# sanderslab/magellanmapper

Hardware: AMD Instinct MI355X
Metric: Mvoxels/s, 2048x2048x1024 uint16 stack, 5-sigma LoG blob detection (higher is better)
Workload: dtype f16x2 MFMA (f32 accumulate) + 16-bit fixed-point intermediates; f64 re-score of every candidate

## Files before the change

### magellanmapper_amd/csrc/mmx_ymfma.hip

```cpp

#include <type_traits>

#include <cstdlib>

#include "mmx_device.h"

struct ym_cfg {
    float w2[MMX_MAX_RADIUS_FAST + 1];
    float w0[MMX_MAX_RADIUS_FAST + 1];
    float unscale;
    float start;
    float lo, eps;
    int radius;
    int reverse;
};

namespace {

#ifndef YM5_OCC
#define YM5_OCC 2
#endif
#ifndef YM6_WAVES
#define YM6_WAVES 4
#define YM6_JH 4
#define YM6_NF 4
#endif
template <int NB, bool MASK>
__global__ void __launch_bounds__(NB <= 4 ? 256 : YM6_WAVES * 64, NB <= 4 ? 3 : (YM6_WAVES == 4 ? YM5_OCC : 1))
ym_kernel(const mmx_block* __restrict__ blocks, int64_t slot_elems, int64_t tile_stride,
          const unsigned* __restrict__ gt, float* __restrict__ out, ym_cfg cfg,
          unsigned long long* __restrict__ mask)
{
    constexpr int RB = 8 * (NB - 2);
    constexpr int NF = NB <= 4 ? 4 : YM6_NF;
    __shared__ v4u frag[NB * NF * 64];
    constexpr int WAVES = NB <= 4 ? 4 : YM6_WAVES;
    constexpr int JH = NB <= 4 ? 4 : YM6_JH;
    __shared__ float tr[WAVES * 2 * 1024];

    const mmx_block bd = blocks[cfg.reverse ? gridDim.y - 1 - blockIdx.y : blockIdx.y];
    const int ntx = (bd.nx + 15) >> 4, ntz = (bd.nz + 15) >> 4;
    if ((int)blockIdx.x * (WAVES / 4) >= ntx * ntz) return;
    for (int e = threadIdx.x; e < NB * NF * 64; e += WAVES * 64) {
        const int ln = e & 63, f = e >> 6;
        const int piece = (f % NF) % (NF / 2), kern = (f % NF) / (NF / 2), t = f / NF;
        const int m = ln & 15, kq = ln >> 4;
        const int delta = RB - 16 * t;
        unsigned pk[4];
#pragma unroll
        for (int i = 0; i < 8; i += 2) {
            float v[2];
#pragma unroll
            for (int u = 0; u < 2; ++u) {
                int d = 8 * kq + i + u - m + delta;
                d = d < 0 ? -d : d;
                const float ws = d <= cfg.radius ? (kern ? cfg.w0[d] : cfg.w2[d]) : 0.f;
                const float h = (float)(_Float16)ws;
                v[u] = piece == 0 ? h : (piece == 1 ? (ws - h) * 256.f : h * 256.f);
            }
            pk[i >> 1] = pack_h2(v[0], v[1]);
        }
        frag[e] = (v4u){pk[0], pk[1], pk[2], pk[3]};
    }
    __syncthreads();

    const int wv = __builtin_amdgcn_readfirstlane((int)(threadIdx.x >> 6));
    const int tile = (int)blockIdx.x * (WAVES / 4) + (wv >> 2);
    if (tile >= ntx * ntz) return;
    const int c = tile / ntz, U = tile - c * ntz;
    const int zq = wv & 3;
    if (16 * U + 4 * zq >= bd.nz) return;
    const int lane = threadIdx.x & 63;
    const int n = bd.ny;
    const float nms_lo = cfg.lo, nms_eps = cfg.eps, us = cfg.unscale;
    const int kq = lane >> 4, n16 = lane & 15;
    const unsigned trow_b = (unsigned)(ntx * ntz) * 1024u;
    const rsrc_t rs = make_rsrc(gt + (int64_t)bd.slot * tile_stride + (int64_t)tile * 256);
    const unsigned voff = (unsigned)(zq * 256 + n16 * 16);
    const unsigned voff_s = voff + (unsigned)(8 * kq) * trow_b;
    const int xi = lane & 15;
    const int z = 16 * U + 4 * zq + (lane >> 4), x = 16 * c + xi;
    const bool real = z < bd.nz && x < bd.nx;
    float* w1 = out + (int64_t)bd.slot * slot_elems;
    const rsrc_t rsw = make_rsrc(w1);
    const unsigned ooff = (unsigned)((real ? z : 0) * bd.ny * bd.px + (real ? x : 0)) * 4u;
    const unsigned row_b = (unsigned)bd.px * 4u;
    const mmx_entry_geom eg = mmx_entry_geom_make(MMX_MASK_QUADS, bd.nz, bd.nx, bd.px);
    const int nent = eg.per_row;
    ulonglong2* mrow = MASK ? reinterpret_cast<ulonglong2*>(mask) + mmx_entry_base(bd.slot, slot_elems) +
                              mmx_quads_entry(eg, 4 * U + zq, 0) + c
                            : nullptr;
    unsigned long long ab_prev = 0;
    const bool has_l = xi > 0, has_r = xi < 15 && x + 1 < bd.nx;
    float prev1 = -INFINITY, prev2 = -INFINITY, nbx_prev = -INFINITY;
    int ydone = 0;
    float* trw = tr + wv * 2048;

    auto close_pending = [&]() __attribute__((always_inline)) {
        unsigned long long m = 0;
        if (ab_prev) {
            const bool cand = real & (prev1 > nms_lo) & !(fmaxf(prev2, nbx_prev) > prev1 + nms_eps);
            m = __ballot(cand);
        }
        if (lane == 0) *mrow = make_ulonglong2(m, ab_prev);
    };
    auto row = [&](float acc, int y) __attribute__((always_inline)) {
        const unsigned long long ab = MASK ? mmx_above_word(real, acc, nms_lo) : ~0ull;
#ifndef YM_NOSTORE
        if (ab && real) __builtin_amdgcn_raw_buffer_store_b32(__float_as_uint(acc * us), rsw, ooff, (unsigned)y * row_b, 0);
#endif
        if constexpr (MASK) {
            float nbx = -INFINITY;
            if (ab) {
                nbx = mmx_x_neighbours<false>(acc, has_l, has_r);
            }
            if (ydone > 0) {
                unsigned long long m = 0;
                if (ab_prev) {
                    const bool cand = real & (prev1 > nms_lo) & !(fmaxf(fmaxf(prev2, acc), nbx_prev) > prev1 + nms_eps);
                    m = __ballot(cand);
                }
                if (lane == 0) *mrow = make_ulonglong2(m, ab_prev);
                mrow += nent;
            }
            prev2 = prev1; prev1 = acc; nbx_prev = nbx;
            ab_prev = ab;
            ++ydone;
        }
    };
    auto rows_of = [&](int T, int s, bool any) __attribute__((always_inline)) {
        if (T < 0 || 16 * T >= n) return;
        const int cnt = n - 16 * T < 16 ? n - 16 * T : 16;
        if (MASK && !any) {
            if (ydone > 0) {
                close_pending();
                mrow += nent;
            }
            if (lane < cnt - 1) mrow[(int64_t)lane * nent] = make_ulonglong2(0ull, 0ull);
            mrow += (int64_t)(cnt - 1) * nent;
            prev1 = prev2 = nbx_prev = -INFINITY;
            ab_prev = 0;
            ydone += cnt;
            return;
        }
        const float* src = trw + s * 1024 + lane;
        if (!MASK || cnt < 16) {
#pragma unroll 1
            for (int r = 0; r < cnt; ++r) row(src[r * 64], 16 * T + r);
            return;
        }
        float v[16];
#pragma unroll
        for (int r = 0; r < 16; ++r) v[r] = src[r * 64];
        unsigned long long ab[16];
        unsigned long long some = 0;
#pragma unroll
        for (int r = 0; r < 16; ++r) { ab[r] = mmx_above_word(real, v[r], nms_lo); some |= ab[r]; }
        unsigned e0 = 0, e1 = 0, e2 = 0, e3 = 0;
        auto put = [&](int ln, unsigned long long m, unsigned long long a) __attribute__((always_inline)) {
            const bool me = lane == ln;
            e0 = me ? (unsigned)m : e0;
            e1 = me ? (unsigned)(m >> 32) : e1;
            e2 = me ? (unsigned)a : e2;
            e3 = me ? (unsigned)(a >> 32) : e3;
        };
        if (ab_prev) {
            const bool cand = real & (prev1 > nms_lo) & !(fmaxf(fmaxf(prev2, v[0]), nbx_prev) > prev1 + nms_eps);
            put(0, __ballot(cand), ab_prev);
        }
        float nbx15 = -INFINITY;
        if (some) {
#pragma unroll
            for (int r = 0; r < 16; ++r) {
                if (ab[r]) {
#ifndef YM_NOSTORE
                    if (real) __builtin_amdgcn_raw_buffer_store_b32(__float_as_uint(v[r] * us), rsw, ooff, (unsigned)(16 * T + r) * row_b, 0);
#endif
                    const float nbx = mmx_x_neighbours<false>(v[r], has_l, has_r);
                    if (r < 15) {
                        const float below = r > 0 ? v[r > 0 ? r - 1 : 0] : prev1;
                        const bool cand = real & (v[r] > nms_lo) & !(fmaxf(fmaxf(below, v[r < 15 ? r + 1 : 15]), nbx) > v[r] + nms_eps);
                        put(r + 1, __ballot(cand), ab[r]);
                    } else {
                        nbx15 = nbx;
                    }
                }
            }
        }
        if (lane < 16 && (lane > 0 || ydone > 0)) {
            ulonglong2* dst = mrow + (int64_t)(ydone > 0 ? lane : lane - 1) * nent;
            *dst = make_ulonglong2((unsigned long long)e0 | ((unsigned long long)e1 << 32),
                                   (unsigned long long)e2 | ((unsigned long long)e3 << 32));
        }
        mrow += (int64_t)(ydone > 0 ? 16 : 15) * nent;
        prev2 = v[14]; prev1 = v[15]; nbx_prev = nbx15;
        ab_prev = ab[15];
        ydone += 16;
    };

#ifndef YM_PFD
#define YM_PFD 1
#endif
    constexpr int PFD = YM_PFD;
    v4u rawA[8], rawB[PFD == 2 ? 8 : 1];
    auto load_block = [&](int b, v4u (&raw)[8]) __attribute__((always_inline)) {
        const int r0 = -RB + 32 * b;
        if (r0 >= 0 && r0 + 32 <= n) {
#pragma unroll
            for (int i = 0; i < 8; ++i)
                raw[i] = __builtin_bit_cast(v4u, __builtin_amdgcn_raw_buffer_load_b128(rs, voff_s, (unsigned)(r0 + i) * trow_b, 0));
        } else {
#pragma unroll
            for (int i = 0; i < 8; ++i) {
                int v = r0 + 8 * kq + i;
                v = v < 0 ? -1 - v : v;
                v = v >= n ? 2 * n - 1 - v : v;
                v = v < 0 ? 0 : (v > n - 1 ? n - 1 : v);
                raw[i] = __builtin_bit_cast(v4u, __builtin_amdgcn_raw_buffer_load_b128(rs, voff + (unsigned)v * trow_b, 0, 0));
            }
        }
    };
    const int nT = (n + 15) >> 4;
    const int nKB = (nT + NB - 3) / 2 + 1;
    const v4f start = {cfg.start, cfg.start, cfg.start, cfg.start};
    v4f acc[NB][4];
#pragma unroll
    for (int t = 0; t < NB; ++t)
#pragma unroll
        for (int j = 0; j < 4; ++j) acc[t][j] = start;
    bool any0 = false, any1 = false;

    const _Float16 k256 = (_Float16)256.f;
    auto iter = [&](int b, v4u (&raw)[8]) __attribute__((always_inline)) {
#ifndef YM_ROWS_LATE
#define YM_ROWS_LATE 1
#endif
        if (!YM_ROWS_LATE || b == nKB) {
#pragma unroll 1
            for (int h = 0; h < 2; ++h) rows_of(2 * (b - 1) - NB + 2 + h, h, h ? any1 : any0);
        }
        if (b == nKB) return false;
        if constexpr (JH < 4) { any0 = !MASK; any1 = !MASK; }
#pragma unroll
        for (int j0 = 0; j0 < 4; j0 += JH) {
            __builtin_amdgcn_sched_barrier(0);
            v4u pc[JH][4];
#pragma unroll
            for (int j = 0; j < JH; ++j)
#pragma unroll
                for (int p = 0; p < 4; ++p) {
                    const unsigned d0 = raw[2 * p][j0 + j], d1 = raw[2 * p + 1][j0 + j];
                    pc[j][0][p] = __builtin_amdgcn_perm(d1, d0, 0x0c050c01u);
                    pc[j][1][p] = __builtin_amdgcn_perm(d1, d0, 0x0c040c00u);
                    pc[j][2][p] = __builtin_amdgcn_perm(d1, d0, 0x0c070c03u) ^ 0x00800080u;
                    pc[j][3][p] = __builtin_amdgcn_perm(d1, d0, 0x0c060c02u);
                }
            __builtin_amdgcn_sched_barrier(0);
            if (j0 + JH == 4 && b + PFD < nKB) load_block(b + PFD, raw);
            __builtin_amdgcn_sched_barrier(0);
            if (YM_ROWS_LATE && JH == 4) {
#pragma unroll 1
                for (int h = 0; h < 2; ++h) rows_of(2 * (b - 1) - NB + 2 + h, h, h ? any1 : any0);
                __builtin_amdgcn_sched_barrier(0);
            }
            auto tile_mfmas = [&](int t, bool fresh) __attribute__((always_inline)) {
                v4f* a = &acc[t][j0];
                const v4u* fr = frag + (t * NF) * 64 + lane;
                const v4u ah = fr[0], al = fr[64], bh = fr[(NF / 2) * 64], bl = fr[(NF / 2 + 1) * 64];
                const v4u a256 = NF == 6 ? fr[128] : __builtin_bit_cast(v4u, __builtin_bit_cast(v8h, ah) * k256);
                const v4u b256 = NF == 6 ? fr[320] : __builtin_bit_cast(v4u, __builtin_bit_cast(v8h, bh) * k256);
#pragma unroll
                for (int j = 0; j < JH; ++j) a[j] = mfma16(a256, pc[j][0], fresh ? start : a[j]);
#pragma unroll
                for (int j = 0; j < JH; ++j) a[j] = mfma16(ah, pc[j][1], a[j]);
#pragma unroll
                for (int j = 0; j < JH; ++j) a[j] = mfma16(al, pc[j][0], a[j]);
#pragma unroll
                for (int j = 0; j < JH; ++j) a[j] = mfma16(b256, pc[j][2], a[j]);
#pragma unroll
                for (int j = 0; j < JH; ++j) a[j] = mfma16(bh, pc[j][3], a[j]);
#pragma unroll
                for (int j = 0; j < JH; ++j) a[j] = mfma16(bl, pc[j][2], a[j]);
            };
#pragma unroll
            for (int t = 0; t < 2; ++t) tile_mfmas(t, t >= NB - 2);
#pragma unroll
            for (int t = 0; t < 2; ++t) {
                const v4f* a = &acc[t][j0];
                float mx = -INFINITY;
#pragma unroll
                for (int j = 0; j < JH; ++j)
#pragma unroll
                    for (int r = 0; r < 4; ++r) mx = fmaxf(mx, a[j][r]);
                const bool any = MASK ? __ballot(mx > nms_lo) != 0ull : true;
                if constexpr (JH == 4) {
                    if (t == 0) any0 = any; else any1 = any;
                    if (any) {
                        v4f* dst = reinterpret_cast<v4f*>(trw + t * 1024) + (4 * kq) * 16 + n16;
#pragma unroll
                        for (int r = 0; r < 4; ++r) dst[r * 16] = (v4f){a[0][r], a[1][r], a[2][r], a[3][r]};
                    }
                } else {
                    if (t == 0) any0 |= any; else any1 |= any;
                    v2f* dst = reinterpret_cast<v2f*>(trw + t * 1024) + (4 * kq) * 32 + 2 * n16 + (j0 >> 1);
#pragma unroll
                    for (int r = 0; r < 4; ++r) dst[r * 32] = (v2f){a[0][r], a[1][r]};
                }
            }
            __builtin_amdgcn_sched_barrier(0);
#pragma unroll
            for (int t = 2; t < NB; ++t) {
                tile_mfmas(t, t >= NB - 2);
                if constexpr (NB > 4) __builtin_amdgcn_sched_barrier(0);
            }
        }
#pragma unroll
        for (int t = 0; t + 2 < NB; ++t)
#pragma unroll
            for (int j = 0; j < 4; ++j) acc[t][j] = acc[t + 2][j];
        __builtin_amdgcn_wave_barrier();
        return true;
    };
    load_block(0, rawA);
    if constexpr (PFD == 2) {
        if (nKB > 1) load_block(1, reinterpret_cast<v4u (&)[8]>(rawB));
#pragma unroll 1
        for (int b = 0;; b += 2) {
            if (!iter(b, rawA)) break;
            if (!iter(b + 1, reinterpret_cast<v4u (&)[8]>(rawB))) break;
        }
    } else {
#pragma unroll 1
        for (int b = 0; iter(b, rawA); ++b) {}
    }
    if constexpr (MASK) close_pending();
}

template <int NB>
int launch_ym(const mmx_block* d_blocks, int n_blocks, const mmx_zx6_plan& plan, int64_t slot_elems,
              const ym_cfg& cfg, const float* d_p, float* d_log, unsigned long long* d_mask, hipStream_t s)
{
    constexpr int TPW = NB <= 4 ? 1 : YM6_WAVES / 4;
    dim3 grid((plan.max_tiles + TPW - 1) / TPW, n_blocks);
    if (d_mask)
        hipLaunchKernelGGL((ym_kernel<NB, true>), grid, dim3(256 * TPW), 0, s, d_blocks, slot_elems, plan.tile_stride,
                           reinterpret_cast<const unsigned*>(d_p), d_log, cfg, d_mask);
    else
        hipLaunchKernelGGL((ym_kernel<NB, false>), grid, dim3(256 * TPW), 0, s, d_blocks, slot_elems, plan.tile_stride,
                           reinterpret_cast<const unsigned*>(d_p), d_log, cfg, d_mask);
    return hipGetLastError() == hipSuccess ? MMX_OK : MMX_ERR_HIP;
}

}

int mmx_launch_ym(const mmx_block* d_blocks, int n_blocks, const mmx_zx6_plan& plan, int64_t slot_elems,
                  const mmx_taps_f32& taps, int radius, const float* d_p, float cp, float cq, float bias,
                  float* d_log, unsigned long long* d_mask, float nms_lo, float nms_eps, hipStream_t stream)
{
    if (!mmx_ym_accepts(taps.w0, taps.w2, radius, cp, cq)) return MMX_ERR_UNSUPPORTED;
    ym_cfg cfg;
    float mx = 0.f;
    for (int k = 0; k <= radius; ++k) {
        cfg.w2[k] = taps.w2[k] * cp;
        cfg.w0[k] = taps.w0[k] * cq;
        mx = fmaxf(mx, fmaxf(fabsf(cfg.w2[k]), fabsf(cfg.w0[k])));
    }
    int e;
    frexpf(mx, &e);
    const float up = ldexpf(1.f, -e - 1);
    double q128 = 0.0;
    for (int k = 0; k <= MMX_MAX_RADIUS_FAST; ++k) {
        cfg.w2[k] = k <= radius ? cfg.w2[k] * up : 0.f;
        cfg.w0[k] = k <= radius ? cfg.w0[k] * up : 0.f;
        const float h = (float)(_Float16)cfg.w0[k];
        const float l = (float)(_Float16)((cfg.w0[k] - h) * 256.f);
        q128 += (k ? 2.0 : 1.0) * ((double)h * 256.0 + (double)l);
    }
    cfg.unscale = ldexpf(1.f, e + 1 + 24);
    cfg.start = (float)(-128.0 * 0x1p-24 * q128 + (double)bias / (double)cfg.unscale);
    cfg.lo = nms_lo / cfg.unscale;
    cfg.eps = nms_eps / cfg.unscale;
    cfg.radius = radius;
    cfg.reverse = 1;
    if (radius <= 8) return launch_ym<3>(d_blocks, n_blocks, plan, slot_elems, cfg, d_p, d_log, d_mask, stream);
    if (radius <= 16) return launch_ym<4>(d_blocks, n_blocks, plan, slot_elems, cfg, d_p, d_log, d_mask, stream);
    return launch_ym<5>(d_blocks, n_blocks, plan, slot_elems, cfg, d_p, d_log, d_mask, stream);
}
```

Before: 46530.

## Swizzle transpose LDS layout, hoist first block load, ballot-based NMS with DPP

The first input block load now starts before the filter-fragment setup and its barrier, so the load latency overlaps the fragment construction. The accumulator transpose buffer uses an XOR-swizzled v4f layout, which allows 128-bit LDS stores and loads in place of scalar strided ones. The full-tile NMS path builds per-row above and beaten masks from wave-wide ballots and DPP neighbour shifts, and writes entries with v_writelane instead of select chains. The PFD=2 prefetch option is removed, the loop is restructured so the last rows are drained after it, and the next block is always prefetched, which may issue an extra out-of-range load at the end.

```diff
diff --git a/magellanmapper_amd/csrc/mmx_ymfma.hip b/magellanmapper_amd/csrc/mmx_ymfma.hip
--- a/magellanmapper_amd/csrc/mmx_ymfma.hip
+++ b/magellanmapper_amd/csrc/mmx_ymfma.hip
@@ -16,6 +16,15 @@
 };
 
 namespace {
+
+template <int LN>
+__device__ __forceinline__ unsigned ym_writelane(unsigned v, unsigned s)
+{
+    asm("v_writelane_b32 %0, %1, %2" : "+v"(v) : "s"(s), "n"(LN));
+    return v;
+}
+
+__device__ __forceinline__ int ym_hput(int lane) { return (lane << 2) | ((lane >> 2) & 3); }
 
 #ifndef YM5_OCC
 #define YM5_OCC 2
@@ -41,6 +50,40 @@
     const mmx_block bd = blocks[cfg.reverse ? gridDim.y - 1 - blockIdx.y : blockIdx.y];
     const int ntx = (bd.nx + 15) >> 4, ntz = (bd.nz + 15) >> 4;
     if ((int)blockIdx.x * (WAVES / 4) >= ntx * ntz) return;
+    const int wv = __builtin_amdgcn_readfirstlane((int)(threadIdx.x >> 6));
+    const int tile = (int)blockIdx.x * (WAVES / 4) + (wv >> 2);
+    const int c = tile / ntz, U = tile - c * ntz;
+    const int zq = wv & 3;
+    const bool live = tile < ntx * ntz && 16 * U + 4 * zq < bd.nz;
+    const int lane = threadIdx.x & 63;
+    const int n = bd.ny;
+    const int kq = lane >> 4, n16 = lane & 15;
+    const unsigned trow_b = (unsigned)(ntx * ntz) * 1024u;
+    const rsrc_t rs = make_rsrc(gt + (int64_t)bd.slot * tile_stride + (int64_t)tile * 256);
+    const unsigned voff = (unsigned)(zq * 256 + n16 * 16);
+    const unsigned voff_s = voff + (unsigned)(8 * kq) * trow_b;
+    v4u raw[8];
+    auto load_block = [&](int b) __attribute__((always_inline)) {
+        const int r0 = -RB + 32 * b;
+        if (r0 >= 0 && r0 + 32 <= n) {
+#pragma unroll
+            for (int i = 0; i < 8; ++i)
+                raw[i] = __builtin_bit_cast(v4u, __builtin_amdgcn_raw_buffer_load_b128(rs, voff_s, (unsigned)(r0 + i) * trow_b, 0));
+        } else {
+            int ln;
+            asm volatile("v_mbcnt_lo_u32_b32 %0, -1, 0\n\tv_mbcnt_hi_u32_b32 %0, -1, %0" : "=v"(ln));
+            const int k8 = (ln >> 1) & 24;
+#pragma unroll
+            for (int i = 0; i < 8; ++i) {
+                int v = r0 + k8 + i;
+                v = v < 0 ? -1 - v : v;
+                v = v >= n ? 2 * n - 1 - v : v;
+                v = v < 0 ? 0 : (v > n - 1 ? n - 1 : v);
+                raw[i] = __builtin_bit_cast(v4u, __builtin_amdgcn_raw_buffer_load_b128(rs, voff + (unsigned)v * trow_b, 0, 0));
+            }
+        }
+    };
+    if (live) load_block(0);
     for (int e = threadIdx.x; e < NB * NF * 64; e += WAVES * 64) {
         const int ln = e & 63, f = e >> 6;
         const int piece = (f % NF) % (NF / 2), kern = (f % NF) / (NF / 2), t = f / NF;
@@ -64,20 +107,8 @@
     }
     __syncthreads();
 
-    const int wv = __builtin_amdgcn_readfirstlane((int)(threadIdx.x >> 6));
-    const int tile = (int)blockIdx.x * (WAVES / 4) + (wv >> 2);
-    if (tile >= ntx * ntz) return;
-    const int c = tile / ntz, U = tile - c * ntz;
-    const int zq = wv & 3;
-    if (16 * U + 4 * zq >= bd.nz) return;
-    const int lane = threadIdx.x & 63;
-    const int n = bd.ny;
+    if (!live) return;
     const float nms_lo = cfg.lo, nms_eps = cfg.eps, us = cfg.unscale;
-    const int kq = lane >> 4, n16 = lane & 15;
-    const unsigned trow_b = (unsigned)(ntx * ntz) * 1024u;
-    const rsrc_t rs = make_rsrc(gt + (int64_t)bd.slot * tile_stride + (int64_t)tile * 256);
-    const unsigned voff = (unsigned)(zq * 256 + n16 * 16);
-    const unsigned voff_s = voff + (unsigned)(8 * kq) * trow_b;
     const int xi = lane & 15;
     const int z = 16 * U + 4 * zq + (lane >> 4), x = 16 * c + xi;
     const bool real = z < bd.nz && x < bd.nx;
@@ -92,9 +123,12 @@
                             : nullptr;
     unsigned long long ab_prev = 0;
     const bool has_l = xi > 0, has_r = xi < 15 && x + 1 < bd.nx;
+    const unsigned long long realw = __builtin_amdgcn_ballot_w64(real), has_lw = __builtin_amdgcn_ballot_w64(has_l),
+                             has_rw = __builtin_amdgcn_ballot_w64(has_r);
     float prev1 = -INFINITY, prev2 = -INFINITY, nbx_prev = -INFINITY;
     int ydone = 0;
-    float* trw = tr + wv * 2048;
+    v4f* trw = reinterpret_cast<v4f*>(tr + wv * 2048);
+    const int hget = lane ^ (lane >> 4);
 
     auto close_pending = [&]() __attribute__((always_inline)) {
         unsigned long long m = 0;
@@ -136,57 +170,81 @@
                 close_pending();
                 mrow += nent;
             }
-            if (lane < cnt - 1) mrow[(int64_t)lane * nent] = make_ulonglong2(0ull, 0ull);
+            int ln = lane;
+            asm volatile("" : "+v"(ln));
+            if (ln < cnt - 1) mrow[(int64_t)ln * nent] = make_ulonglong2(0ull, 0ull);
             mrow += (int64_t)(cnt - 1) * nent;
             prev1 = prev2 = nbx_prev = -INFINITY;
             ab_prev = 0;
             ydone += cnt;
             return;
         }
-        const float* src = trw + s * 1024 + lane;
-        if (!MASK || cnt < 16) {
-#pragma unroll 1
-            for (int r = 0; r < cnt; ++r) row(src[r * 64], 16 * T + r);
+        const v4f* src = trw + s * 256 + hget;
+        if constexpr (!MASK) {
+#pragma unroll 1
+            for (int g = 0; 4 * g < cnt; ++g) {
+                const v4f q = src[g * 64];
+#pragma unroll
+                for (int r = 0; r < 4; ++r)
+                    if (4 * g + r < cnt) row(q[r], 16 * T + 4 * g + r);
+            }
             return;
         }
+        if (cnt < 16) {
+            const float* src1 = reinterpret_cast<const float*>(src);
+#pragma unroll 1
+            for (int r = 0; r < cnt; ++r) row(src1[(r >> 2) * 256 + (r & 3)], 16 * T + r);
+            return;
+        }
         float v[16];
 #pragma unroll
-        for (int r = 0; r < 16; ++r) v[r] = src[r * 64];
-        unsigned long long ab[16];
-        unsigned long long some = 0;
-#pragma unroll
-        for (int r = 0; r < 16; ++r) { ab[r] = mmx_above_word(real, v[r], nms_lo); some |= ab[r]; }
+        for (int g = 0; g < 4; ++g) {
+            const v4f q = src[g * 64];
+#pragma unroll
+            for (int r = 0; r < 4; ++r) v[4 * g + r] = q[r];
+        }
         unsigned e0 = 0, e1 = 0, e2 = 0, e3 = 0;
-        auto put = [&](int ln, unsigned long long m, unsigned long long a) __attribute__((always_inline)) {
-            const bool me = lane == ln;
-            e0 = me ? (unsigned)m : e0;
-            e1 = me ? (unsigned)(m >> 32) : e1;
-            e2 = me ? (unsigned)a : e2;
-            e3 = me ? (unsigned)(a >> 32) : e3;
+        auto put = [&](auto LN, unsigned long long beaten, unsigned long long a) __attribute__((always_inline)) {
+            constexpr int ln = decltype(LN)::value;
+            const unsigned long long m = a & ~beaten;
+            e0 = ym_writelane<ln>(e0, (unsigned)m);
+            e1 = ym_writelane<ln>(e1, (unsigned)(m >> 32));
+            e2 = ym_writelane<ln>(e2, (unsigned)a);
+            e3 = ym_writelane<ln>(e3, (unsigned)(a >> 32));
         };
-        if (ab_prev) {
-            const bool cand = real & (prev1 > nms_lo) & !(fmaxf(fmaxf(prev2, v[0]), nbx_prev) > prev1 + nms_eps);
-            put(0, __ballot(cand), ab_prev);
-        }
+        if (ab_prev)
+            put(std::integral_constant<int, 0>{},
+                __builtin_amdgcn_ballot_w64(fmaxf(fmaxf(prev2, v[0]), nbx_prev) > prev1 + nms_eps), ab_prev);
         float nbx15 = -INFINITY;
-        if (some) {
-#pragma unroll
-            for (int r = 0; r < 16; ++r) {
-                if (ab[r]) {
+        unsigned long long ab15 = 0;
+        auto one = [&](auto R) __attribute__((always_inline)) {
+            constexpr int r = decltype(R)::value;
+            const unsigned long long ab_r = __builtin_amdgcn_ballot_w64(v[r] > nms_lo) & realw;
+            if constexpr (r == 15) ab15 = ab_r;
+            if (ab_r) {
 #ifndef YM_NOSTORE
-                    if (real) __builtin_amdgcn_raw_buffer_store_b32(__float_as_uint(v[r] * us), rsw, ooff, (unsigned)(16 * T + r) * row_b, 0);
+                if (real) __builtin_amdgcn_raw_buffer_store_b32(__float_as_uint(v[r] * us), rsw, ooff, (unsigned)(16 * T + r) * row_b, 0);
 #endif
-                    const float nbx = mmx_x_neighbours<false>(v[r], has_l, has_r);
-                    if (r < 15) {
-                        const float below = r > 0 ? v[r > 0 ? r - 1 : 0] : prev1;
-                        const bool cand = real & (v[r] > nms_lo) & !(fmaxf(fmaxf(below, v[r < 15 ? r + 1 : 15]), nbx) > v[r] + nms_eps);
-                        put(r + 1, __ballot(cand), ab[r]);
-                    } else {
-                        nbx15 = nbx;
-                    }
+                if constexpr (r < 15) {
+                    const float below = r > 0 ? v[r > 0 ? r - 1 : 0] : prev1;
+                    const float t = v[r] + nms_eps;
+                    const int b = (int)__float_as_uint(v[r]);
+                    const float l = __uint_as_float((unsigned)__builtin_amdgcn_update_dpp(0, b, 0x111 , 0xf, 0xf, true));
+                    const float rr = __uint_as_float((unsigned)__builtin_amdgcn_update_dpp(0, b, 0x101 , 0xf, 0xf, true));
+                    put(std::integral_constant<int, r + 1>{},
+                        __builtin_amdgcn_ballot_w64(below > t) | __builtin_amdgcn_ballot_w64(v[r < 15 ? r + 1 : 15] > t) |
+                            (__builtin_amdgcn_ballot_w64(l > t) & has_lw) | (__builtin_amdgcn_ballot_w64(rr > t) & has_rw),
+                        ab_r);
+                } else {
+                    nbx15 = mmx_x_neighbours<false>(v[r], has_l, has_r);
                 }
             }
-        }
+        };
+        auto each = [&](auto... R) __attribute__((always_inline)) { (one(R), ...); };
+#define YM_R(i) std::integral_constant<int, i>{}
+        each(YM_R(0), YM_R(1), YM_R(2), YM_R(3), YM_R(4), YM_R(5), YM_R(6), YM_R(7), YM_R(8), YM_R(9), YM_R(10), YM_R(11),
+             YM_R(12), YM_R(13), YM_R(14), YM_R(15));
+#undef YM_R
         if (lane < 16 && (lane > 0 || ydone > 0)) {
             ulonglong2* dst = mrow + (int64_t)(ydone > 0 ? lane : lane - 1) * nent;
             *dst = make_ulonglong2((unsigned long long)e0 | ((unsigned long long)e1 << 32),
@@ -194,32 +252,10 @@
         }
         mrow += (int64_t)(ydone > 0 ? 16 : 15) * nent;
         prev2 = v[14]; prev1 = v[15]; nbx_prev = nbx15;
-        ab_prev = ab[15];
+        ab_prev = ab15;
         ydone += 16;
     };
 
-#ifndef YM_PFD
-#define YM_PFD 1
-#endif
-    constexpr int PFD = YM_PFD;
-    v4u rawA[8], rawB[PFD == 2 ? 8 : 1];
-    auto load_block = [&](int b, v4u (&raw)[8]) __attribute__((always_inline)) {
-        const int r0 = -RB + 32 * b;
-        if (r0 >= 0 && r0 + 32 <= n) {
-#pragma unroll
-            for (int i = 0; i < 8; ++i)
-                raw[i] = __builtin_bit_cast(v4u, __builtin_amdgcn_raw_buffer_load_b128(rs, voff_s, (unsigned)(r0 + i) * trow_b, 0));
-        } else {
-#pragma unroll
-            for (int i = 0; i < 8; ++i) {
-                int v = r0 + 8 * kq + i;
-                v = v < 0 ? -1 - v : v;
-                v = v >= n ? 2 * n - 1 - v : v;
-                v = v < 0 ? 0 : (v > n - 1 ? n - 1 : v);
-                raw[i] = __builtin_bit_cast(v4u, __builtin_amdgcn_raw_buffer_load_b128(rs, voff + (unsigned)v * trow_b, 0, 0));
-            }
-        }
-    };
     const int nT = (n + 15) >> 4;
     const int nKB = (nT + NB - 3) / 2 + 1;
     const v4f start = {cfg.start, cfg.start, cfg.start, cfg.start};
@@ -231,15 +267,14 @@
     bool any0 = false, any1 = false;
 
     const _Float16 k256 = (_Float16)256.f;
-    auto iter = [&](int b, v4u (&raw)[8]) __attribute__((always_inline)) {
+    auto iter = [&](int b) __attribute__((always_inline)) {
 #ifndef YM_ROWS_LATE
 #define YM_ROWS_LATE 1
 #endif
-        if (!YM_ROWS_LATE || b == nKB) {
+        if (!YM_ROWS_LATE) {
 #pragma unroll 1
             for (int h = 0; h < 2; ++h) rows_of(2 * (b - 1) - NB + 2 + h, h, h ? any1 : any0);
         }
-        if (b == nKB) return false;
         if constexpr (JH < 4) { any0 = !MASK; any1 = !MASK; }
 #pragma unroll
         for (int j0 = 0; j0 < 4; j0 += JH) {
@@ -255,8 +290,12 @@
                     pc[j][2][p] = __builtin_amdgcn_perm(d1, d0, 0x0c070c03u) ^ 0x00800080u;
                     pc[j][3][p] = __builtin_amdgcn_perm(d1, d0, 0x0c060c02u);
                 }
+#pragma unroll
+            for (int j = 0; j < JH; ++j)
+#pragma unroll
+                for (int k = 0; k < 4; ++k) asm volatile("" : "+v"(pc[j][k]));
             __builtin_amdgcn_sched_barrier(0);
-            if (j0 + JH == 4 && b + PFD < nKB) load_block(b + PFD, raw);
+            if (j0 + JH == 4) load_block(b + 1);
             __builtin_amdgcn_sched_barrier(0);
             if (YM_ROWS_LATE && JH == 4) {
 #pragma unroll 1
@@ -296,15 +335,16 @@
                 if constexpr (JH == 4) {
                     if (t == 0) any0 = any; else any1 = any;
                     if (any) {
-                        v4f* dst = reinterpret_cast<v4f*>(trw + t * 1024) + (4 * kq) * 16 + n16;
-#pragma unroll
-                        for (int r = 0; r < 4; ++r) dst[r * 16] = (v4f){a[0][r], a[1][r], a[2][r], a[3][r]};
+                        int ln = lane;
+                        asm volatile("" : "+v"(ln));
+                        const int hp = ym_hput(ln);
+#pragma unroll
+                        for (int j = 0; j < 4; ++j) trw[t * 256 + (hp ^ j)] = a[j];
                     }
                 } else {
                     if (t == 0) any0 |= any; else any1 |= any;
-                    v2f* dst = reinterpret_cast<v2f*>(trw + t * 1024) + (4 * kq) * 32 + 2 * n16 + (j0 >> 1);
-#pragma unroll
-                    for (int r = 0; r < 4; ++r) dst[r * 32] = (v2f){a[0][r], a[1][r]};
+#pragma unroll
+                    for (int j = 0; j < JH; ++j) trw[t * 256 + (ym_hput(lane) ^ (j0 + j))] = a[j];
                 }
             }
             __builtin_amdgcn_sched_barrier(0);
@@ -319,20 +359,11 @@
 #pragma unroll
             for (int j = 0; j < 4; ++j) acc[t][j] = acc[t + 2][j];
         __builtin_amdgcn_wave_barrier();
-        return true;
     };
-    load_block(0, rawA);
-    if constexpr (PFD == 2) {
-        if (nKB > 1) load_block(1, reinterpret_cast<v4u (&)[8]>(rawB));
-#pragma unroll 1
-        for (int b = 0;; b += 2) {
-            if (!iter(b, rawA)) break;
-            if (!iter(b + 1, reinterpret_cast<v4u (&)[8]>(rawB))) break;
-        }
-    } else {
-#pragma unroll 1
-        for (int b = 0; iter(b, rawA); ++b) {}
-    }
+#pragma unroll 1
+    for (int b = 0; b < nKB; ++b) iter(b);
+#pragma unroll 1
+    for (int h = 0; h < 2; ++h) rows_of(2 * (nKB - 1) - NB + 2 + h, h, h ? any1 : any0);
     if constexpr (MASK) close_pending();
 }
 
```

New measurement: 47210, median of 6. 1.5% higher.
